# nucypher/SGFHE.jl

Hardware: AMD Instinct MI355X
Metric: bootstraps/sec (higher is better)
Workload: dtype i32

## Files before the change

sgfhe.jl_amd/csrc/engine.hip:

```cpp
#include "../../include/sgfhe_hip.h"

#include <math.h>
#include <stdio.h>
#include <stdlib.h>
#include <string.h>

#include <atomic>
#include <chrono>
#include <condition_variable>
#include <deque>
#include <memory>
#include <mutex>
#include <string>
#include <thread>
#include <type_traits>
#include <unordered_map>
#include <vector>

#include "kernels.h"
#include "host_plumbing.h"
#include "coalescer.h"
#include "circuit.h"

using namespace sgfhe;
// ... 74 lines not shown

struct SharedDev {
    int device = 0;
    std::mutex mu;
    std::vector<void *> mem;
    Coalescer co;
    std::atomic<unsigned> clones{0};
    void own(void *p) {
        std::lock_guard<std::mutex> g(mu);
        mem.push_back(p);
    }
    ~SharedDev() {
        (void)hipSetDevice(device);
        for (void *p : mem) (void)hipFree(p);
    }
};

struct sgfhe_ctx {
    sgfhe_params par;
    int device = 0;
    int logm = 0;
    uint32_t M = 0, n = 0;
    u128 Q = 0, B = 0;
    struct Basis {
        uint32_t npr = 0;
        uint32_t primes[NPR_MAX] = {};
        PrimeK *d_primes = nullptr;
        CrtConst *d_crt = nullptr;
        CrtConst h_crt;
        CrtLean *d_lean = nullptr;
        CrtLean h_lean;
        bool lean_rnd_ok = false;
        uint32_t pack_G = 1, pack_G_rnd = 0;
        int32_t *d_key = nullptr;
        size_t key_bytes = 0;
    } basis[2];
    int nb = 1, active = 0;
    uint32_t npr_max = 0;
    uint32_t tw_done = 0;
    std::string err;
    std::shared_ptr<SharedDev> shared;
    mutable std::recursive_mutex mu;
    hipStream_t stream = nullptr;
    hipStream_t stream2 = nullptr;
    hipEvent_t ev_fork = nullptr, ev_join = nullptr;
    hipEvent_t ev_done = nullptr;
    bool pending = false;
    hipStream_t stream_io = nullptr, stream_io2 = nullptr;
    std::vector<hipEvent_t> ev_pool;
    uint32_t *d_bad = nullptr;
    int32_t *d_tw = nullptr;
    int32_t *d_twq = nullptr;
    int32_t *d_pow = nullptr;
    int32_t tw_head[NPR_MAX][8] = {};
    uint32_t fused_min = 7;
    uint32_t split_max = 7;
    bool have_key = false;
    uint32_t chunk = 0, cap = 0, lanes = 2;
    bool rnd = false, rnd_ok = false;
    ChaChaKey rnd_key = {};
    uint32_t rnd_call = 0, last_call = 0;
    int64_t call_fixed = -1;
    const RndRow *gather_rows = nullptr;
    DevBuf<RndRow> d_rows;
    std::vector<RndRow> h_rows;
    uint32_t create_flags = 0;
    bool have_rns2 = false;
    Rns2Const rns2;
    struct Lane {
        uint64_t *dig = nullptr;
        uint32_t *yres = nullptr;
        uint32_t *ua = nullptr;
        int32_t *zpart = nullptr;
    } lane[2];
    bool small_padded = false;
    bool small_lanes = true;
    uint32_t small_lanes_max = 24;
    uint32_t crt1_max = 0;
    uint32_t small_max = 24;
    DevBuf<uint64_t> io_in, io_out;
    DevBuf<uint64_t, true> pin_in, pin_out;
    std::vector<uint64_t> co_buf;
    bool use_pin = true;
    DevBuf<uint64_t> circ_wires, circ_stage, circ_out;
    DevBuf<uint32_t> circ_tab;
    DevBuf<uint64_t> circ_ct;
    DevBuf<uint64_t> pack_lwe, pack_pdig, pack_wv;
    DevBuf<ulonglong2> pack_raw;
    DevBuf<uint32_t> pack_yg;
    DevBuf<ulonglong2> circ_raw;
    DevBuf<uint64_t> noise_tab, noise_lwe;
    bool timing = false;
    struct EvTriple { hipEvent_t e0, e1, e2; };
    std::vector<EvTriple> ev;
    double t_ext = 0, t_crt = 0;
    uint64_t n_ext = 0, n_crt = 0;
    uint32_t last_chunk = 0;
    struct EvPair { hipEvent_t e0, e1; uint64_t batch; };
    std::vector<EvPair> ev_call;
    double t_call = 0;
    uint64_t n_call = 0, boots_call = 0;
    uint32_t attr_done = 0;
};
enum : uint32_t { ATTR_EXTPROD = 1u, ATTR_SMALL = 2u, ATTR_SHORTPROD = 4u, ATTR_FUSED = 8u };
static constexpr size_t PIN_MAX_BYTES = (size_t)1 << 30;
static size_t pin_max_bytes() {
// ... 67 lines not shown
enum class ExtKind {
    Throughput,
    Small,
    Quarter,
    Fused
};
struct ExtForm {
    ExtKind kind;
    uint32_t cnt;
    bool quarter() const { return kind == ExtKind::Quarter || kind == ExtKind::Fused; }
};
ExtForm ext_form(const sgfhe_ctx *c, uint32_t mode, uint32_t cb, uint32_t cpad, bool has_zpart) {
    const bool small = cpad <= c->small_max && has_zpart;
    const uint32_t cnt = small && !c->small_padded ? cb : cpad;
    if (small && cnt >= c->fused_min && cnt <= fused_cap(c, mode)) return {ExtKind::Fused, cnt};
    if (small && quarter_ok(c, mode) && cnt <= c->split_max) return {ExtKind::Quarter, cnt};
    return {small ? ExtKind::Small : ExtKind::Throughput, cnt};
}

enum class CrtKind { Lean, LeanRnd, Acc2, Acc };
struct CrtForm {
    CrtKind kind;
    uint32_t np, nl;
    bool wide;
    bool rows;
    bool p87;
    bool one;
    bool quarter;
    uint32_t per_thread() const { return kind == CrtKind::Acc2 ? 2u : (kind == CrtKind::Acc || one) ? 1u : 4u; }
};
CrtForm crt_form(const sgfhe_ctx *c, uint32_t mode, uint32_t total, bool rows, bool quarter = false) {
    const sgfhe_ctx::Basis &S = cur(c);
    CrtForm f = {CrtKind::Acc, S.npr, S.h_lean.nl, false, false, false, false, quarter};
    if (quarter) {
        f.kind = (mode & MODE_RANDOM) ? CrtKind::LeanRnd : CrtKind::Lean;
        f.one = true;
    } else if (mode == 0u && S.h_lean.nl != 0) {
        f.kind = CrtKind::Lean;
        f.one = total <= c->crt1_max;
        f.p87 = !f.one && S.npr == 5 && S.h_lean.p87;
    } else if ((mode & ~MODE_WIDE) == MODE_RANDOM && S.lean_rnd_ok) {
        f.kind = CrtKind::LeanRnd;
        f.wide = (mode & MODE_WIDE) != 0;
        f.one = !f.wide && total <= c->crt1_max;
    } else if (mode == 0u) {
        f.kind = CrtKind::Acc2;
    }
    f.rows = rows && (f.kind == CrtKind::LeanRnd || f.kind == CrtKind::Acc);
    return f;
}

size_t lds_bytes(int logm, int npoly) { return (size_t)npoly * ((size_t)4 << logm); }
template <int LOGM> constexpr int ext_loge() { return LOGM <= EXT_LE3_MAX ? 3 : LOGE; }
template <int LOGM> constexpr int threads_of() { return NttGeom<LOGM, LOGE>::T; }


template <class F> int32_t with_logm(sgfhe_ctx *c, F &&f) {
    switch (c->logm) {
#define X(LM) case LM: return f(std::integral_constant<int, LM>{});
        X(6) X(7) X(8) X(9) X(10) X(11) X(12) X(13) X(14)
#undef X
    }
    return fail(c, SGFHE_ERR_UNSUPPORTED, "unsupported log2(m)");
}
template <class F> int32_t with_npr(sgfhe_ctx *c, uint32_t npr, F &&f) {
    switch (npr) {
#define X(NP) case NP: return f(std::integral_constant<int, NP>{});
        X(2) X(3) X(4) X(5) X(6) X(7)
#undef X
    }
    return fail(c, SGFHE_ERR_UNSUPPORTED, "unsupported number of RNS primes");
}
template <class F> void with_nl(uint32_t nl, F &&f) {
    switch (nl) {
    case 2: f(std::integral_constant<int, 2>{}); break;
    case 3: f(std::integral_constant<int, 3>{}); break;
    default: f(std::integral_constant<int, 4>{}); break;
    }
}
template <class F> void with_bool(bool b, F &&f) {
    if (b) f(std::true_type{});
    else f(std::false_type{});
}


int32_t launch_extprod(sgfhe_ctx *c, const sgfhe_ctx::Lane &L, const int32_t *keyk, uint32_t cpad,
                       uint32_t k, uint32_t mode, hipStream_t st) {
    return with_logm(c, [&](auto lm) -> int32_t {
        constexpr int LOGM = decltype(lm)::value, LE = ext_loge<LOGM>();
        const size_t lds = lds_bytes(LOGM, 2);
        if (!(c->attr_done & ATTR_EXTPROD)) {
            HIPCHK(c, hipFuncSetAttribute((const void *)k_extprod<LOGM, LE, false>,
                                          hipFuncAttributeMaxDynamicSharedMemorySize, (int)lds));
            HIPCHK(c, hipFuncSetAttribute((const void *)k_extprod<LOGM, LE, true>,
                                          hipFuncAttributeMaxDynamicSharedMemorySize, (int)lds));
            c->attr_done |= ATTR_EXTPROD;
        }
        with_bool(mode & MODE_WIDE, [&](auto wide) {
            hipLaunchKernelGGL((k_extprod<LOGM, LE, decltype(wide)::value>), dim3(cpad * cur(c).npr),
                               dim3(NttGeom<LOGM, LE>::T), lds, st, L.dig, keyk, L.yres, L.ua, cur(c).d_primes, k,
                               c->n, mode);
        });
        HIPCHK(c, hipGetLastError());
        return SGFHE_OK;
    });
}
// ... 683 lines not shown
    std::vector<int32_t> tw((size_t)NPR * 4 * M), twq, pwt;
    std::vector<PrimeK> pk(NPR);
    cc.npr = npr;
    for (int i = 0; i < NPR; i++) {
        const uint32_t p = S.primes[i];
        if ((uint32_t)i >= c->tw_done) {
        uint32_t psi = 0;
        for (uint32_t x = 2; x < 2000 && !psi; x++) {
            uint32_t g = powmod32(x, (p - 1) / (2 * M), p);
            if (powmod32(g, M, p) == p - 1) psi = g;
        }
        if (!psi) return fail(c, SGFHE_ERR_UNSUPPORTED, "no primitive 2m-th root of unity");
        const uint32_t ipsi = powmod32(psi, p - 2, p);
        int32_t *f = tw.data() + (size_t)(4 * i) * M, *v = f + M, *fp = f + 2 * M, *vp = f + 3 * M;
        const uint32_t R1m = (uint32_t)((1ull << 32) % p);
        std::vector<uint32_t> pf(M), pv(M);
        uint32_t pw = 1, ipw = 1;
        for (uint32_t t = 0; t < M; t++) {
            const uint32_t br = bitrev(t, logm);
            pf[br] = pw;
            pv[br] = ipw;
            f[br] = centre32(mulmod32(pw, R1m, p), p);
            v[br] = centre32(mulmod32(ipw, R1m, p), p);
            pw = mulmod32(pw, psi, p);
            ipw = mulmod32(ipw, ipsi, p);
        }
        fp[0] = fp[1] = vp[0] = vp[1] = 0;
        for (uint32_t j = 2; j < M; j++) {
            const uint32_t a = mulmod32(mulmod32(pf[j >> 1], pf[j], p), R1m, p);
            const uint32_t b = mulmod32(mulmod32(pv[j >> 1], pv[j], p), R1m, p);
            fp[j] = centre32((j & 1) ? (p - a) % p : a, p);
            vp[j] = centre32((j & 1) ? (p - b) % p : b, p);
        }
        if (M >= 16) {
            const uint32_t MS = M / 4;
            twq.assign((size_t)4 * M, 0);
            for (uint32_t q = 0; q < 4; q++)
                for (uint32_t jj = 1; jj < MS; jj++) {
                    const uint32_t mmq = 1u << (31 - __builtin_clz(jj)), J = 4 * mmq + q * mmq + (jj - mmq);
                    int32_t *blk = twq.data() + (size_t)q * M;
                    blk[jj] = f[J];
                    blk[MS + jj] = v[J];
                    blk[2 * MS + jj] = jj >= 2 ? fp[J] : 0;
                    blk[3 * MS + jj] = jj >= 2 ? vp[J] : 0;
                }
            HIPCHK(c, hipMemcpy(c->d_twq + (size_t)(4 * i) * M, twq.data(), (size_t)4 * M * sizeof(int32_t), hipMemcpyHostToDevice));
        }
        {
            pwt.resize((size_t)2 * M);
            uint32_t pe = 1;
            for (uint32_t e = 0; e < 2 * M; e++) { pwt[e] = centre32(mulmod32(pe, R1m, p), p); pe = mulmod32(pe, psi, p); }
            HIPCHK(c, hipMemcpy(c->d_pow + (size_t)(2 * i) * M, pwt.data(), (size_t)2 * M * sizeof(int32_t), hipMemcpyHostToDevice));
        }
        const int32_t head[8] = {f[1], M > 2 ? f[2] : 0, M > 2 ? f[3] : 0, M > 2 ? fp[2] : 0, M > 2 ? fp[3] : 0,
                                 v[1], M > 2 ? v[2] : 0, M > 2 ? v[3] : 0};
        memcpy(c->tw_head[i], head, sizeof head);
        }
        PrimeK &P = pk[i];
        memset(&P, 0, sizeof P);
        P.p = (int32_t)p;
        uint32_t inv = p;
        for (int it = 0; it < 5; it++) inv *= 2u - p * inv;
        P.pinv = inv;
        const uint32_t R1 = (uint32_t)((1ull << 32) % p);
        const uint32_t Rinv = powmod32(R1, p - 2, p);
        const uint32_t R2 = mulmod32(R1, R1, p);
        P.r1 = centre32(R1, p);
        P.r2 = centre32(R2, p);
        P.r3 = centre32(mulmod32(R2, R1, p), p);
        P.sR = centre32((p - mulmod32((uint32_t)(s % p), Rinv, p)) % p, p);
        {
            const u128 xmax = (B & 1) ? (B - 1) / 2 * 3 : B / 2 * 3;
            P.sRr = centre32((p - mulmod32((uint32_t)((s + xmax) % p), Rinv, p)) % p, p);
        }
        P.hoff = (i == NPR - 1) ? (p - 1) / 2 : 0;
        P.qmodp = centre32((uint32_t)(Q % p), p);
        uint32_t Mi = 1;
        for (int j = 0; j < NPR; j++)
            if (j != i) Mi = mulmod32(Mi, S.primes[j] % p, p);
        const uint32_t ei = powmod32(Mi, p - 2, p);
        const uint32_t minv = powmod32(M % p, p - 2, p);
        const uint32_t kappa = mulmod32(mulmod32(R2, minv, p), ei, p);
        P.kappaR = centre32(mulmod32(kappa, R1, p), p);
        P.minvR = centre32(mulmod32(minv, R1, p), p);
        P.invp = 1.0f / (float)p;
        P.twf = c->d_tw + (size_t)(4 * i) * M;
        P.twi = c->d_tw + (size_t)(4 * i + 1) * M;
        P.npr = npr;
        P.f1 = c->tw_head[i][0]; P.f2 = c->tw_head[i][1]; P.f3 = c->tw_head[i][2];
        P.fp2 = c->tw_head[i][3]; P.fp3 = c->tw_head[i][4];
        P.v1 = c->tw_head[i][5]; P.v2 = c->tw_head[i][6]; P.v3 = c->tw_head[i][7];
        P.twq = c->d_twq + (size_t)(4 * i) * M;
        P.pw = c->d_pow + (size_t)(2 * i) * M;
    }
    if (c->tw_done < npr) {
        const size_t off = (size_t)c->tw_done * 4 * M;
        HIPCHK(c, hipMemcpy(c->d_tw + off, tw.data() + off, ((size_t)npr * 4 * M - off) * sizeof(int32_t),
                            hipMemcpyHostToDevice));
        c->tw_done = npr;
    }
    HIPCHK(c, hipMalloc(&S.d_primes, NPR * sizeof(PrimeK)));
    c->shared->own(S.d_primes);
    HIPCHK(c, hipMemcpy(S.d_primes, pk.data(), NPR * sizeof(PrimeK), hipMemcpyHostToDevice));
    HIPCHK(c, hipMalloc(&S.d_crt, sizeof(CrtConst)));
    c->shared->own(S.d_crt);
    HIPCHK(c, hipMemcpy(S.d_crt, &cc, sizeof(CrtConst), hipMemcpyHostToDevice));
    HIPCHK(c, hipMalloc(&S.d_lean, sizeof(CrtLean)));
    c->shared->own(S.d_lean);
    HIPCHK(c, hipMemcpy(S.d_lean, &S.h_lean, sizeof(CrtLean), hipMemcpyHostToDevice));
    return SGFHE_OK;
}

int32_t build_constants(sgfhe_ctx *c) {
    const int logm = c->logm;
    const u128 Q = c->Q, B = c->B;

    uint32_t cand_primes[NPR_MAX];
    {
        int found = 0;
        for (uint64_t kk = ((1ull << 29) - 1) >> 15; kk > 0 && found < NPR_MAX; kk--) {
            uint32_t cand = (uint32_t)((kk << 15) + 1);
            if (cand < (1u << 29) && is_prime32(cand)) cand_primes[found++] = cand;
        }
        if (found < NPR_MAX) return fail(c, SGFHE_ERR_UNSUPPORTED, "could not find RNS primes");
    }
    const double log_mbq = logm + u128_log2(B) + u128_log2(Q);
    const double log_need = log2(5.0) + log_mbq + 0.001;
    auto fewest = [&](double target, double *have) {
        uint32_t npr = 0;
        double lh = 0;
        while (npr < NPR_MAX && (npr < 2 || lh < target)) lh += log2((double)cand_primes[npr++]);
        *have = lh;
        return lh >= target ? npr : 0u;
    };
    double have_det = 0, have_rnd = 0;
    const uint32_t npr_det = fewest(log_need, &have_det);
    if (!npr_det)
        return fail(c, SGFHE_ERR_UNSUPPORTED, "5 m B Q exceeds the product of the RNS primes");
    const bool rnd_width_ok = 2.0 * u128_log2(B) + 2.0 - u128_log2(Q) < 50.0;
    const uint32_t npr_rnd = fewest(log_need + 2.0, &have_rnd);
    const bool det_only = (c->create_flags & SGFHE_CTX_DETERMINISTIC_ONLY) != 0;
    c->nb = (!det_only && rnd_width_ok && npr_rnd > npr_det) ? 2 : 1;
    c->rnd_ok = rnd_width_ok && npr_rnd != 0 && (c->nb == 2 || npr_rnd == npr_det);
    c->npr_max = c->nb == 2 ? npr_rnd : npr_det;
    {
        const char *env = getenv("SGFHE_HOST_PIN");
        c->use_pin = !(env && env[0] == '0');
        env = getenv("SGFHE_SMALL_PADDED");
        c->small_padded = env && env[0] == '1';
        env = getenv("SGFHE_SMALL_LANES");
        if (env) { c->small_lanes = atoi(env) != 0; if (atoi(env) > 1) c->small_lanes_max = (uint32_t)atoi(env); }
        env = getenv("SGFHE_CRT1_GATES");
        c->crt1_max = (uint32_t)(env ? atoi(env) : 8) * 2u * c->M;
        if (c->logm >= 14) { c->small_max = 16; if (c->small_lanes_max > 16) c->small_lanes_max = 16; }
    }
    HIPCHK(c, hipMalloc(&c->d_tw, (size_t)c->npr_max * 4 * c->M * sizeof(int32_t)));
    c->shared->own(c->d_tw);
    HIPCHK(c, hipMalloc(&c->d_twq, (size_t)c->npr_max * 4 * c->M * sizeof(int32_t)));
    c->shared->own(c->d_twq);
    HIPCHK(c, hipMalloc(&c->d_pow, (size_t)c->npr_max * 2 * c->M * sizeof(int32_t)));
    c->shared->own(c->d_pow);
    {
        const char *env = getenv("SGFHE_SMALL_SPLIT");
        if (env) c->split_max = (uint32_t)atoi(env);
        env = getenv("SGFHE_SMALL_FUSED");
        if (env) c->fused_min = (uint32_t)atoi(env);
    }
    HIPCHK(c, hipMalloc(&c->d_bad, sizeof(uint32_t)));
    HIPCHK(c, hipMemset(c->d_bad, 0, sizeof(uint32_t)));
    for (int b = c->nb - 1; b >= 0; b--) {
        const bool big = b == c->nb - 1 && c->nb == 2;
        int32_t rc = build_basis(c, c->basis[b], big ? npr_rnd : npr_det, cand_primes, big ? have_rnd : have_det, log_mbq);
        if (rc) return rc;
    }
    c->active = 0;
    return SGFHE_OK;
}

int32_t key_begin(sgfhe_ctx *c) {
    if (c->shared.use_count() > 1)
        return fail(c, SGFHE_ERR_INVALID_ARG,
                    "the bootstrap key of this ctx is shared with clones (sgfhe_ctx_clone): destroy them before replacing it");
    c->active = c->nb - 1;
    return SGFHE_OK;
}
sgfhe_ctx::Basis &key_basis(sgfhe_ctx *c) { return c->basis[c->nb - 1]; }
void key_dirty(sgfhe_ctx *c) { c->have_key = false; }
int32_t key_finish(sgfhe_ctx *c, int32_t rc) {
    if (rc == SGFHE_OK && c->nb == 2) {
        const sgfhe_ctx::Basis &Bg = c->basis[1];
        sgfhe_ctx::Basis &Sm = c->basis[0];
        hipError_t e = hipSuccess;
        if (!Sm.d_key) {
            Sm.key_bytes = (size_t)c->n * Sm.npr * 8 * c->M * 4;
            e = hipMalloc(&Sm.d_key, Sm.key_bytes);
            if (e == hipSuccess) c->shared->own(Sm.d_key);
        }
        if (e == hipSuccess) {
            KeyFactors fac = {};
            for (uint32_t i = 0; i < Sm.npr; i++) {
                const uint32_t p = Sm.primes[i];
                uint32_t f = (uint32_t)((1ull << 32) % p);
                for (uint32_t j = Sm.npr; j < Bg.npr; j++) f = mulmod32(f, Bg.primes[j] % p, p);
                fac.f[i] = centre32(f, p);
            }
            const size_t total = Sm.key_bytes / 4;
            hipLaunchKernelGGL(k_key_derive, dim3((unsigned)((total + 255) / 256)), dim3(256), 0, c->stream,
                               Bg.d_key, Sm.d_key, Sm.d_primes, fac, Bg.npr, Sm.npr, (uint32_t)c->logm, total);
            e = hipGetLastError();
            if (e == hipSuccess) e = hipStreamSynchronize(c->stream);
        }
        if (e != hipSuccess) { rc = fail(c, SGFHE_ERR_HIP, hipGetErrorString(e)); c->have_key = false; }
    }
    c->active = mode_basis(c);
// ... 132 lines not shown
    {
        const char *env = getenv("SGFHE_COALESCE");
        if (env && env[0] == '0') c->shared->co.enabled = false;
    }
    const uint64_t m = p->m;
    if (p->ell != 2) return fail(c, SGFHE_ERR_UNSUPPORTED, "ell must be 2 (fhe.jl:576)");
    if (m < 64 || m > 16384 || (m & (m - 1)))
        return fail(c, SGFHE_ERR_UNSUPPORTED, "m must be a power of two in [2^6, 2^14]");
    if (p->r != 2 * m) return fail(c, SGFHE_ERR_INVALID_ARG, "r must equal 2 m (fhe.jl:62)");
    if (p->n == 0 || p->n > m / 4 || (p->n & (p->n - 1)))
        return fail(c, SGFHE_ERR_INVALID_ARG,
                    "n must be a power of two in [1, m / 4] (fhe.jl:45-46; extract, fhe.jl:585-590)");
    c->M = (uint32_t)m;
    c->n = (uint32_t)p->n;
    while ((1u << c->logm) < c->M) c->logm++;
    c->Q = ld128(p->Q);
    c->B = ld128(p->B);
    if (c->Q < 3 || (c->Q >> 94)) return fail(c, SGFHE_ERR_UNSUPPORTED, "Q must be in [3, 2^94)");
    if (c->B < 2 || (c->B >> 47)) return fail(c, SGFHE_ERR_UNSUPPORTED, "B must be in [2, 2^47)");
    {
        if (c->B * c->B < c->Q) return fail(c, SGFHE_ERR_INVALID_ARG, "B^2 must be >= Q");
    }
    if (ld128(p->DQ_tilde) >= c->Q) return fail(c, SGFHE_ERR_INVALID_ARG, "DQ_tilde must be < Q");
    int32_t rc = create_streams(c);
    if (rc) return rc;
    return build_constants(c);
}

int32_t sgfhe_ctx_clone(sgfhe_ctx *src, sgfhe_ctx **out) {
    if (!src || !out) return SGFHE_ERR_INVALID_ARG;
    *out = nullptr;
    SGFHE_LOCK(src);
    if (!src->have_key) return fail(src, SGFHE_ERR_NO_KEY, "ctx_clone: the ctx has no bootstrap key to share");
    if (hipSetDevice(src->device) != hipSuccess) return fail(src, SGFHE_ERR_NO_DEVICE, "ctx_clone: hipSetDevice failed");
    sgfhe_ctx *c = new (std::nothrow) sgfhe_ctx();
    if (!c) return fail(src, SGFHE_ERR_OOM, "out of host memory");
    *out = c;
    c->par = src->par;
    c->device = src->device;
    c->logm = src->logm;
    c->M = src->M;
    c->n = src->n;
    c->Q = src->Q;
    c->B = src->B;
    c->create_flags = src->create_flags;
    c->shared = src->shared;
    for (int b = 0; b < 2; b++) c->basis[b] = src->basis[b];
    c->nb = src->nb;
    c->npr_max = src->npr_max;
    c->tw_done = src->tw_done;
    c->d_tw = src->d_tw;
    c->d_twq = src->d_twq;
    c->d_pow = src->d_pow;
    memcpy(c->tw_head, src->tw_head, sizeof c->tw_head);
    c->rnd_ok = src->rnd_ok;
    c->have_rns2 = src->have_rns2;
    c->rns2 = src->rns2;
    c->have_key = true;
    c->chunk = src->chunk;
    c->lanes = src->lanes;
    c->small_max = src->small_max;
    c->small_lanes = src->small_lanes;
    c->small_lanes_max = src->small_lanes_max;
    c->small_padded = src->small_padded;
    c->crt1_max = src->crt1_max;
    c->split_max = src->split_max;
    c->fused_min = src->fused_min;
    c->use_pin = src->use_pin;
    hipStream_t skip[3] = {nullptr, nullptr, nullptr};
    const unsigned shift = c->shared->clones.fetch_add(1) % 4u + 1u;
    for (unsigned i = 0; i < shift % 4u; i++) (void)hipStreamCreateWithFlags(&skip[i], hipStreamNonBlocking);
    int32_t rc = create_streams(c);
    for (hipStream_t x : skip)
        if (x) (void)hipStreamDestroy(x);
    if (rc) return rc;
    HIPCHK(c, hipMalloc(&c->d_bad, sizeof(uint32_t)));
    HIPCHK(c, hipMemset(c->d_bad, 0, sizeof(uint32_t)));
    return SGFHE_OK;
}

static void free_circuit_buffers(sgfhe_ctx *c) {
    c->circ_wires.release();
    c->circ_stage.release();
    c->circ_out.release();
    c->circ_tab.release();
    c->circ_ct.release();
    c->circ_raw.release();
    c->noise_tab.release();
    c->noise_lwe.release();
    c->pack_lwe.release();
    c->pack_raw.release();
    c->pack_pdig.release();
    c->pack_yg.release();
    c->pack_wv.release();
}
static void free_io_buffers(sgfhe_ctx *c) {
    c->io_in.release();
    c->io_out.release();
    c->pin_in.release();
    c->pin_out.release();
}

extern "C++" template <typename T>
static int32_t circ_grow(sgfhe_ctx *c, DevBuf<T> &buf, size_t words) {
    if (buf.grow(words) == hipSuccess) return SGFHE_OK;
    return fail(c, SGFHE_ERR_OOM, "sgfhe_circuit_run: hipMalloc of " + std::to_string(words * sizeof(T)) +
// ... 1602 lines not shown
```

sgfhe.jl_amd/csrc/kernels.h:

```cpp
#pragma once

#include "ntt.h"

namespace sgfhe {

typedef unsigned __int128 u128;

constexpr int NPR_MAX = 7;
constexpr int LOGE = 4;

struct PrimeK {
    int32_t p;
    uint32_t pinv;
    int32_t sR;
    int32_t sRr;
    uint32_t hoff;
    int32_t r1, r2, r3;
    int32_t qmodp;
    int32_t kappaR;
    int32_t minvR;
    float invp;
    const int32_t *twf;
    const int32_t *twi;
    uint32_t npr;
    int32_t f1, f2, f3, fp2, fp3;
    int32_t v1, v2, v3;
    const int32_t *twq;
    const int32_t *pw;
};
__device__ __forceinline__ Mod mod_of(const PrimeK &P) { return Mod{P.p, -P.p, P.pinv}; }

typedef const PrimeK *__restrict__ PrimeSet;

constexpr int CRT_ALPHA_MAX = 6 * NPR_MAX + 2;

struct CrtConst {
    u128 Q, B;
    u128 c[NPR_MAX];
    u128 T[CRT_ALPHA_MAX];
    u128 offneg;
    u128 offneg_rnd;
    uint64_t xmax;
    u128 DQ;
    u128 halfQ;
    u128 roundthr;
    double invQ, invB;
    uint32_t c32[NPR_MAX][3];
    uint32_t Q32[3];
    alignas(16) uint32_t T32[CRT_ALPHA_MAX][4];
    double cd[NPR_MAX], Td[CRT_ALPHA_MAX], Bd;
    float invp[NPR_MAX];
    uint32_t npr;
    uint32_t logr;
    ulonglong2 dig0, digP, digN;
};

enum : uint32_t {
    MODE_PLAIN = 1u,
    MODE_NOACC = 2u,
    MODE_CANON = 4u,
    MODE_RANDOM = 16u,
    MODE_WIDE = 32u
};


__device__ __forceinline__ double u128_to_double(u128 x) {
    return (double)(uint64_t)(x >> 64) * 18446744073709551616.0 + (double)(uint64_t)x;
}
__device__ __forceinline__ u128 mul_u64_u128(uint64_t a, u128 b) {
    return (u128)a * (uint64_t)b + (((u128)(a * (uint64_t)(b >> 64))) << 64);
}
__device__ __forceinline__ u128 mod_wide(u128 x, u128 d, double inv, uint64_t *quot) {
    uint64_t q = (uint64_t)(u128_to_double(x) * inv);
    u128 r = x - mul_u64_u128(q, d);
#pragma unroll 1
    while ((__int128)r < 0) { r += d; q--; }
#pragma unroll 1
    while (r >= d) { r -= d; q++; }
    if (quot) *quot = q;
    return r;
}
// ... 173 lines not shown
    uint32_t q;
    int32_t wB, wP;
    __device__ __forceinline__ QuarterHead(uint32_t q_, const PrimeK &P)
        : q(q_), wB((q_ & 2) ? P.f3 : P.f2), wP((q_ & 2) ? P.fp3 : P.fp2) {}
    template <int MS>
    __device__ __forceinline__ int32_t point(const uint32_t *dl, const uint16_t *dh, uint32_t i, const PrimeK &P,
                                             const Mod &md, int32_t sRd) const {
        int32_t X[4];
#pragma unroll
        for (int t = 0; t < 4; t++)
            X[t] = digit_reduce(dl[i + t * MS] | ((uint64_t)dh[i + t * MS] << 32), md, sRd);
        const int32_t u = smont(X[2], P.f1, md);
        const int32_t a = (q & 2) ? X[0] - u : X[0] + u;
        const int32_t w = sredc((int64_t)X[1] * wB + (int64_t)X[3] * wP, md);
        return sred_floor((q & 1) ? a - w : a + w, md);
    }
};

template <int LOGM, int E>
__device__ __forceinline__ void rot_factors(int32_t (&dfac)[E], const PrimeK &P, uint32_t j, uint32_t q, int t) {
    constexpr uint32_t M = 1u << LOGM;
#pragma unroll
    for (int e = 0; e < E; e++) {
        const uint32_t sl = q * (M / 4) + (uint32_t)(E * t + e);
        const uint32_t br = __brev(sl) >> (32 - LOGM);
        dfac[e] = P.pw[(j * (2u * br + 1u)) & (2u * M - 1u)];
    }
}
__device__ __forceinline__ int32_t rot_centre(int32_t dfac, const PrimeK &P, const Mod &md) {
    return scentre(dfac - P.r1, md);
}

template <int NP>
__device__ __forceinline__ void quarter_residues(const int32_t *__restrict__ ypart, PrimeSet PS, uint32_t bc,
                                                 uint32_t i, uint32_t logm, uint32_t (&y)[NP]) {
    const uint32_t MS = (1u << logm) >> 2, jq = i & (MS - 1), qq = i >> (logm - 2);
#pragma unroll
    for (int q = 0; q < NP; q++) {
        const PrimeK P = PS[q];
        const Mod md = mod_of(P);
        const int32_t *yp = ypart + (((size_t)bc * NP + q) * 4) * MS + jq;
        int32_t r;
        if (qq & 1u) {
            const int32_t c1 = smont(yp[0] - yp[MS], P.v2, md), c3 = smont(yp[2 * MS] - yp[3 * MS], P.v3, md);
            r = (qq & 2u) ? smont(c1 - c3, P.v1, md) : c1 + c3;
        } else {
            const int32_t c0 = sred(yp[0] + yp[MS], md), c2 = sred(yp[2 * MS] + yp[3 * MS], md);
            r = (qq & 2u) ? smont(c0 - c2, P.v1, md) : c0 + c2;
        }
        y[q] = (uint32_t)r + handover_offset(P);
    }
}

constexpr int EXT_WAVES = 4;
constexpr int wide_split(int logm) { return logm >= 13 ? 2 : 4; }
constexpr int DET_SPLIT = 0;
constexpr int EXT_LE3_MAX = 9;
template <int LOGM, int LE, bool WIDE = false>
__global__ void __launch_bounds__((NttGeom<LOGM, LE>::T), (NttGeom<LOGM, LE>::T >= 256 ? EXT_WAVES : 1))
k_extprod(const uint64_t *__restrict__ dig, const int32_t *__restrict__ keyk,
          uint32_t *__restrict__ yres, const uint32_t *__restrict__ ua, PrimeSet PS, uint32_t k,
          uint32_t n, uint32_t mode) {
    using G = NttGeom<LOGM, LE>;
    constexpr int M = G::M, T = G::T, E = G::E;
    extern __shared__ __attribute__((aligned(16))) uint32_t lds[];
    int32_t *const z1 = reinterpret_cast<int32_t *>(lds) + M + threadIdx.x;

    const int tid = threadIdx.x;
    const uint32_t g = blockIdx.x;
    const uint32_t slot = g >> 3;
    const uint32_t npr = PS[0].npr;
    const uint32_t b = (slot / npr) * 8 + (g & 7);
    const uint32_t pi = slot % npr;
    const PrimeK P = PS[pi];
    const Mod md = mod_of(P);
    const uint32_t cpad = gridDim.x / npr;
    const BufRsrc rdig = make_rsrc(dig, cpad * 32u * (uint32_t)M);
    const BufRsrc rkey = make_rsrc(keyk, npr * 32u * (uint32_t)M);
#ifdef SGFHE_ABL_NO_YRES
    const BufRsrc ryres = make_rsrc(yres, 0u);
#else
    const BufRsrc ryres = make_rsrc(yres, cpad * npr * 8u * (uint32_t)M);
#endif

    const int32_t sRd = (mode & MODE_RANDOM) ? P.sRr : P.sR;
    constexpr int SPLIT = E == 16 ? (WIDE ? wide_split(LOGM) : DET_SPLIT) : 0;
    int64_t acc0[E];
#pragma unroll
    for (int e = 0; e < E; e++) { acc0[e] = 0; z1[e * T] = 0; }
#pragma unroll 1
    for (int ph = 0; ph < 4; ph++) {
        const int tid = (int)threadIdx.x + (int)opaque_zero();
        int32_t x[1][E];
        const uint32_t srec = (b * 2u + (uint32_t)(ph >> 1)) * 16u * (uint32_t)M;
        const uint32_t slo = srec + (uint32_t)(ph & 1) * 4u * (uint32_t)M;
        const uint32_t shi = srec + 8u * (uint32_t)M + (uint32_t)(ph & 1) * 2u * (uint32_t)M;
        const uint32_t vlo = 4u * (uint32_t)tid, vhi = 2u * (uint32_t)tid;
#pragma unroll
        for (int e = 0; e < E; e++) {
#ifdef SGFHE_ABL_NO_DIG
            x[0][e] = digit_reduce((uint64_t)(tid + e) * 0x9E3779B97F4Aull, md, sRd);
#else
            const uint32_t OL = (uint32_t)(4 * T * e), OH = (uint32_t)(2 * T * e);
            const uint32_t lo = buf_ld_u32(rdig, vlo + (OL & 4095u), slo + (OL & ~4095u));
            uint32_t hi = buf_ld_u16(rdig, vhi + (OH & 4095u), shi + (OH & ~4095u));
            if constexpr (WIDE)
                hi |= buf_ld_u8(rdig, (uint32_t)tid + ((uint32_t)(T * e) & 4095u),
                                srec + 12u * (uint32_t)M + (uint32_t)(ph & 1) * (uint32_t)M + ((uint32_t)(T * e) & ~4095u)) << 16;
            x[0][e] = digit_reduce(lo | ((uint64_t)hi << 32), md, sRd);
#endif
            if constexpr (SPLIT > 1)
                if ((e + 1) % (E / SPLIT) == 0 && e + 1 < E) __builtin_amdgcn_sched_barrier(0);
        }
        SGFHE_SYNC();

        const uint32_t skey = (pi * 8u + (uint32_t)ph * 2u) * 4u * (uint32_t)M;
        const uint32_t vkey = 4u * (uint32_t)E * (uint32_t)tid;
        int4 ka4[E / 4], kb4[E / 4];
        ntt_forward<LOGM, 1, LE>(x, lds, P.twf, tid, md);
#pragma unroll
        for (int h = 0; h < E / 4; h++) {
#ifdef SGFHE_ABL_NO_KEY
            ka4[h] = make_int4(tid, h, ph, 7), kb4[h] = make_int4(h, tid, 5, ph);
#else
            ka4[h] = buf_ld_i4(rkey, vkey + 16u * (uint32_t)h, skey);
            kb4[h] = buf_ld_i4(rkey, vkey + 16u * (uint32_t)h, skey + 4u * (uint32_t)M);
#endif
        }

        const Mod &mdp = md;
#pragma unroll
        for (int h = 0; h < E / 4; h++) {
            const int4 a = ka4[h], bq = kb4[h];
            const int32_t ka[4] = {a.x, a.y, a.z, a.w};
            const int32_t kb[4] = {bq.x, bq.y, bq.z, bq.w};
#pragma unroll
            for (int t = 0; t < 4; t++) {
                const int e = 4 * h + t;
                const int32_t u = x[0][e];
                acc0[e] += (int64_t)u * ka[t];
                int32_t *zp = reinterpret_cast<int32_t *>(lds) + M + e * T + tid;
                *zp += smont(u, kb[t], mdp);
            }
        }
    }
    int32_t z[2][E];
    constexpr bool WIDE0 = !inv_r4(LOGM) && LE == 4 && NttGeom<LOGM, LE>::SLAST_INV >= 0 &&
                           !(NttGeom<LOGM, LE>::RHO == 0 && NttGeom<LOGM, LE>::STOP == 0);
#pragma unroll
    for (int e = 0; e < E; e++) {
        const int32_t r0 = sredc(acc0[e], md);
        z[0][e] = WIDE0 ? r0 : sred(r0, md);
        z[1][e] = sred(z1[e * T], md);
    }
    SGFHE_SYNC();
    ntt_inverse<LOGM, 2, LE, WIDE0>(z, lds, P.twi, tid, md);

    const uint32_t sy0 = (b * 2u * npr + pi) * 4u * (uint32_t)M;
    const uint32_t sy1 = sy0 + npr * 4u * (uint32_t)M;
    const uint32_t vout = 4u * (uint32_t)tid;
    if (mode & MODE_PLAIN) {
#pragma unroll
        for (int c = 0; c < 2; c++)
#pragma unroll
            for (int e = 0; e < E; e++)
                buf_st_u32(ryres, vout + ((uint32_t)(4 * T * e) & 4095u),
                              (c ? sy1 : sy0) + ((uint32_t)(4 * T * e) & ~4095u),
                              condsub(sfull(z[c][e], md) + P.hoff, (uint32_t)P.p));
        return;
    }
    const uint32_t j = ua[(size_t)b * n + k];
    const uint32_t yoff = handover_offset(P);
    lds_store<LOGM, 2, LE, G::STOP>(z, lds, tid);
    SGFHE_SYNC();
    {
        constexpr uint32_t LOWMASK = (1u << G::STOP) - 1u;
        const uint32_t s0 = ((uint32_t)tid - j) & (2 * M - 1);
        const uint32_t lowswz = swz<LE>(s0 & LOWMASK);
        const uint32_t h0 = s0 >> G::STOP;
#pragma unroll
        for (int e = 0; e < E; e++) {
            const uint32_t he = h0 + e;
            const uint32_t hipart = (he & (E - 1)) << G::STOP;
            const uint32_t addr = hipart ^ lowswz ^ (G::STOP >= 9 ? 0u : swz_bits<LE>(hipart));
            const uint32_t smask = 0u - ((he >> LE) & 1u);
            const uint32_t yoe = yoff - smask;
#pragma unroll
            for (int c = 0; c < 2; c++) {
                const uint32_t v = lds[c * M + addr];
                const uint32_t y = (v ^ smask) + (yoe - (uint32_t)z[c][e]);
                buf_st_u32(ryres, vout + ((uint32_t)(4 * T * e) & 4095u),
                              (c ? sy1 : sy0) + ((uint32_t)(4 * T * e) & ~4095u), y);
            }
        }
    }
}

struct U96 {
    uint32_t w0, w1, w2;
};
__device__ __forceinline__ void mad96(U96 &a, uint32_t y, const uint32_t (&c)[3]) {
    const uint64_t p0 = (uint64_t)y * c[0] + a.w0;
    const uint64_t p1 = (uint64_t)y * c[1] + a.w1 + (p0 >> 32);
    a.w0 = (uint32_t)p0;
    a.w1 = (uint32_t)p1;
    a.w2 = y * c[2] + a.w2 + (uint32_t)(p1 >> 32);
}
template <int NP>
__device__ __forceinline__ U96 crt_reduce(const uint32_t (&y)[NP], const CrtConst *__restrict__ CC,
                                          bool have_old, ulonglong2 d) {
    float f = 0.f;
    double Sd = 0.0;
#pragma unroll
    for (int q = 0; q < NP; q++) {
        f += (float)y[q] * CC->invp[q];
#ifndef SGFHE_ABL_CRT_NOSD
        Sd += (double)y[q] * CC->cd[q];
#endif
    }
    const int alpha = (int)f;
    const uint4 tv = *reinterpret_cast<const uint4 *>(CC->T32[alpha]);
    U96 a = {tv.x, tv.y, tv.z};
    Sd += CC->Td[alpha];
#pragma unroll
    for (int q = 0; q < NP; q++) mad96(a, y[q], CC->c32[q]);
    if (have_old) {
        const uint64_t B = (uint64_t)CC->B;
        const uint32_t h0 = (uint32_t)d.y, h1 = (uint32_t)(d.y >> 32);
        const uint32_t b0 = (uint32_t)B, b1 = (uint32_t)(B >> 32);
        const uint64_t p0 = (uint64_t)h0 * b0 + a.w0 + (uint32_t)d.x;
        const uint64_t p1 = (uint64_t)h0 * b1 + (uint64_t)h1 * b0 + a.w1 + (uint32_t)(d.x >> 32) + (p0 >> 32);
        a.w0 = (uint32_t)p0;
        a.w1 = (uint32_t)p1;
        a.w2 += h1 * b1 + (uint32_t)(p1 >> 32);
#ifndef SGFHE_ABL_CRT_NOSD
        Sd += (double)d.y * CC->Bd + (double)d.x;
#endif
    }
    {
        const uint64_t q1 = (uint64_t)(Sd * CC->invQ);
        const uint32_t qa = (uint32_t)q1, qb = (uint32_t)(q1 >> 32);
        const uint64_t m0 = (uint64_t)qa * CC->Q32[0];
        const uint64_t m1 = (uint64_t)qa * CC->Q32[1] + (uint64_t)qb * CC->Q32[0] + (m0 >> 32);
        const uint32_t m2 = qa * CC->Q32[2] + qb * CC->Q32[1] + (uint32_t)(m1 >> 32);
        const uint64_t r0 = (uint64_t)a.w0 - (uint32_t)m0;
        const uint64_t r1 = (uint64_t)a.w1 - (uint32_t)m1 - ((r0 >> 32) & 1u);
        a.w2 = a.w2 - m2 - (uint32_t)((r1 >> 32) & 1u);
        a.w0 = (uint32_t)r0;
// ... 1544 lines not shown
```

Baseline: 2177.

## Fold negacyclic rotation into NTT domain via precomputed (X^j-1) twiddle table

The external-product kernel used to finish with an LDS store, a barrier, and a rotated re-read that formed X^j*z - z in the coefficient domain. Now each NTT-domain value is multiplied pointwise by a precomputed (psi^e - 1) factor before the inverse NTT, so the output can be stored directly. The factors are loaded from a new per-prime table laid out in rows. This removes an LDS round trip and a sync at the cost of extra global table reads and Montgomery multiplies, and it drops the WIDE0 lazy-reduction path.

```diff
diff --git a/sgfhe.jl_amd/csrc/engine.hip b/sgfhe.jl_amd/csrc/engine.hip
--- a/sgfhe.jl_amd/csrc/engine.hip
+++ b/sgfhe.jl_amd/csrc/engine.hip
@@ -150,6 +150,7 @@
     int32_t *d_tw = nullptr;
     int32_t *d_twq = nullptr;
     int32_t *d_pow = nullptr;
+    int32_t *d_rot = nullptr;
     int32_t tw_head[NPR_MAX][8] = {};
     uint32_t fused_min = 7;
     uint32_t split_max = 7;
@@ -323,6 +324,7 @@
 
 size_t lds_bytes(int logm, int npoly) { return (size_t)npoly * ((size_t)4 << logm); }
 template <int LOGM> constexpr int ext_loge() { return LOGM <= EXT_LE3_MAX ? 3 : LOGE; }
+uint32_t rot_row_words(int logm) { return 1u << (logm <= EXT_LE3_MAX ? 3 : LOGE); }
 template <int LOGM> constexpr int threads_of() { return NttGeom<LOGM, LOGE>::T; }
 
 
@@ -1112,6 +1114,16 @@
             for (uint32_t e = 0; e < 2 * M; e++) { pwt[e] = centre32(mulmod32(pe, R1m, p), p); pe = mulmod32(pe, psi, p); }
             HIPCHK(c, hipMemcpy(c->d_pow + (size_t)(2 * i) * M, pwt.data(), (size_t)2 * M * sizeof(int32_t), hipMemcpyHostToDevice));
         }
+        {
+            const uint32_t E = rot_row_words(logm), rows = 2 * M / E;
+            pwt.assign((size_t)2 * M + E, centre32(R1m, p));
+            uint32_t pe = 1;
+            for (uint32_t e = 0; e < 2 * M; e++) {
+                pwt[(size_t)(e % rows) * E + e / rows] = centre32(mulmod32((pe + p - 1) % p, R1m, p), p);
+                pe = mulmod32(pe, psi, p);
+            }
+            HIPCHK(c, hipMemcpy(c->d_rot + (size_t)i * (2 * M + E), pwt.data(), pwt.size() * sizeof(int32_t), hipMemcpyHostToDevice));
+        }
         const int32_t head[8] = {f[1], M > 2 ? f[2] : 0, M > 2 ? f[3] : 0, M > 2 ? fp[2] : 0, M > 2 ? fp[3] : 0,
                                  v[1], M > 2 ? v[2] : 0, M > 2 ? v[3] : 0};
         memcpy(c->tw_head[i], head, sizeof head);
@@ -1152,6 +1164,7 @@
         P.v1 = c->tw_head[i][5]; P.v2 = c->tw_head[i][6]; P.v3 = c->tw_head[i][7];
         P.twq = c->d_twq + (size_t)(4 * i) * M;
         P.pw = c->d_pow + (size_t)(2 * i) * M;
+        P.rot = c->d_rot + (size_t)i * (2 * M + rot_row_words(logm));
     }
     if (c->tw_done < npr) {
         const size_t off = (size_t)c->tw_done * 4 * M;
@@ -1220,6 +1233,8 @@
     c->shared->own(c->d_twq);
     HIPCHK(c, hipMalloc(&c->d_pow, (size_t)c->npr_max * 2 * c->M * sizeof(int32_t)));
     c->shared->own(c->d_pow);
+    HIPCHK(c, hipMalloc(&c->d_rot, (size_t)c->npr_max * (2 * c->M + rot_row_words(c->logm)) * sizeof(int32_t)));
+    c->shared->own(c->d_rot);
     {
         const char *env = getenv("SGFHE_SMALL_SPLIT");
         if (env) c->split_max = (uint32_t)atoi(env);
@@ -1458,6 +1473,7 @@
     c->d_tw = src->d_tw;
     c->d_twq = src->d_twq;
     c->d_pow = src->d_pow;
+    c->d_rot = src->d_rot;
     memcpy(c->tw_head, src->tw_head, sizeof c->tw_head);
     c->rnd_ok = src->rnd_ok;
     c->have_rns2 = src->have_rns2;
diff --git a/sgfhe.jl_amd/csrc/kernels.h b/sgfhe.jl_amd/csrc/kernels.h
--- a/sgfhe.jl_amd/csrc/kernels.h
+++ b/sgfhe.jl_amd/csrc/kernels.h
@@ -27,6 +27,7 @@
     int32_t v1, v2, v3;
     const int32_t *twq;
     const int32_t *pw;
+    const int32_t *rot;
 };
 __device__ __forceinline__ Mod mod_of(const PrimeK &P) { return Mod{P.p, -P.p, P.pinv}; }
 
@@ -306,6 +307,23 @@
     }
 }
 
+template <int LOGM, int LE>
+struct RotRow {
+    static constexpr int E = 1 << LE, LOGROWS = LOGM + 1 - LE;
+    BufRsrc rrot;
+    uint32_t j, row, h4;
+    __device__ __forceinline__ RotRow(const PrimeK &P, uint32_t j_, int tid, bool plain)
+        : rrot(make_rsrc(P.rot, (8u << LOGM) + 4u * E)), j(j_) {
+        const uint32_t jd = j * (2u * (__brev((uint32_t)tid) >> (32 - (LOGM - LE))) + 1u);
+        row = plain ? (8u << LOGM) : (jd & ((1u << LOGROWS) - 1u)) * (4u * E);
+        h4 = (jd >> LOGROWS) << 2;
+    }
+    __device__ __forceinline__ int32_t load(int e) const {
+        const uint32_t se4 = (j * (__brev((uint32_t)e) >> (32 - LE))) << 2;
+        return (int32_t)buf_ld_u32(rrot, row | ((h4 + se4) & (4u * E - 4u)), 0u);
+    }
+};
+
 constexpr int EXT_WAVES = 4;
 constexpr int wide_split(int logm) { return logm >= 13 ? 2 : 4; }
 constexpr int DET_SPLIT = 0;
@@ -338,6 +356,7 @@
 #endif
 
     const int32_t sRd = (mode & MODE_RANDOM) ? P.sRr : P.sR;
+    const uint32_t j = ua[(size_t)b * n + k];
     constexpr int SPLIT = E == 16 ? (WIDE ? wide_split(LOGM) : DET_SPLIT) : 0;
     int64_t acc0[E];
 #pragma unroll
@@ -398,17 +417,16 @@
             }
         }
     }
+    const RotRow<LOGM, LE> rot(P, j, tid + (int)opaque_zero(), (mode & MODE_PLAIN) != 0);
     int32_t z[2][E];
-    constexpr bool WIDE0 = !inv_r4(LOGM) && LE == 4 && NttGeom<LOGM, LE>::SLAST_INV >= 0 &&
-                           !(NttGeom<LOGM, LE>::RHO == 0 && NttGeom<LOGM, LE>::STOP == 0);
 #pragma unroll
     for (int e = 0; e < E; e++) {
-        const int32_t r0 = sredc(acc0[e], md);
-        z[0][e] = WIDE0 ? r0 : sred(r0, md);
-        z[1][e] = sred(z1[e * T], md);
+        const int32_t f = rot.load(e);
+        z[0][e] = smont(sredc(acc0[e], md), f, md);
+        z[1][e] = smont(z1[e * T], f, md);
     }
     SGFHE_SYNC();
-    ntt_inverse<LOGM, 2, LE, WIDE0>(z, lds, P.twi, tid, md);
+    ntt_inverse<LOGM, 2, LE>(z, lds, P.twi, tid, md);
 
     const uint32_t sy0 = (b * 2u * npr + pi) * 4u * (uint32_t)M;
     const uint32_t sy1 = sy0 + npr * 4u * (uint32_t)M;
@@ -423,31 +441,13 @@
                               condsub(sfull(z[c][e], md) + P.hoff, (uint32_t)P.p));
         return;
     }
-    const uint32_t j = ua[(size_t)b * n + k];
     const uint32_t yoff = handover_offset(P);
-    lds_store<LOGM, 2, LE, G::STOP>(z, lds, tid);
-    SGFHE_SYNC();
-    {
-        constexpr uint32_t LOWMASK = (1u << G::STOP) - 1u;
-        const uint32_t s0 = ((uint32_t)tid - j) & (2 * M - 1);
-        const uint32_t lowswz = swz<LE>(s0 & LOWMASK);
-        const uint32_t h0 = s0 >> G::STOP;
-#pragma unroll
-        for (int e = 0; e < E; e++) {
-            const uint32_t he = h0 + e;
-            const uint32_t hipart = (he & (E - 1)) << G::STOP;
-            const uint32_t addr = hipart ^ lowswz ^ (G::STOP >= 9 ? 0u : swz_bits<LE>(hipart));
-            const uint32_t smask = 0u - ((he >> LE) & 1u);
-            const uint32_t yoe = yoff - smask;
-#pragma unroll
-            for (int c = 0; c < 2; c++) {
-                const uint32_t v = lds[c * M + addr];
-                const uint32_t y = (v ^ smask) + (yoe - (uint32_t)z[c][e]);
-                buf_st_u32(ryres, vout + ((uint32_t)(4 * T * e) & 4095u),
-                              (c ? sy1 : sy0) + ((uint32_t)(4 * T * e) & ~4095u), y);
-            }
-        }
-    }
+#pragma unroll
+    for (int c = 0; c < 2; c++)
+#pragma unroll
+        for (int e = 0; e < E; e++)
+            buf_st_u32(ryres, vout + ((uint32_t)(4 * T * e) & 4095u),
+                          (c ? sy1 : sy0) + ((uint32_t)(4 * T * e) & ~4095u), (uint32_t)z[c][e] + yoff);
 }
 
 struct U96 {
```

After: 2105. -3.3%, worse.

## Pair digit phases in external product with parked NTT and joint reduction

Applied to the files above, without the earlier changes.

Restructures the external-product accumulation loop so two digit phases are processed per pass. The first phase's forward-NTT output is parked in LDS and combined with the second's in a single 64-bit multiply-add pair, followed by one Montgomery reduction per output per pair. This replaces the 64-bit accumulator plus a per-element LDS read-modify-write with smont for the second component. The goal is to cut reductions and LDS traffic. In exchange the kernel drops the WIDE0 inverse-NTT path, adds an LDS park store and reload, and puts an extra sred between reductions that may change numeric bounds.

```diff
diff --git a/sgfhe.jl_amd/csrc/kernels.h b/sgfhe.jl_amd/csrc/kernels.h
--- a/sgfhe.jl_amd/csrc/kernels.h
+++ b/sgfhe.jl_amd/csrc/kernels.h
@@ -318,7 +318,7 @@
     using G = NttGeom<LOGM, LE>;
     constexpr int M = G::M, T = G::T, E = G::E;
     extern __shared__ __attribute__((aligned(16))) uint32_t lds[];
-    int32_t *const z1 = reinterpret_cast<int32_t *>(lds) + M + threadIdx.x;
+    int32_t *const park = reinterpret_cast<int32_t *>(lds) + M + threadIdx.x;
 
     const int tid = threadIdx.x;
     const uint32_t g = blockIdx.x;
@@ -339,76 +339,76 @@
 
     const int32_t sRd = (mode & MODE_RANDOM) ? P.sRr : P.sR;
     constexpr int SPLIT = E == 16 ? (WIDE ? wide_split(LOGM) : DET_SPLIT) : 0;
-    int64_t acc0[E];
-#pragma unroll
-    for (int e = 0; e < E; e++) { acc0[e] = 0; z1[e * T] = 0; }
+    int32_t s0[E], s1[E];
+#pragma unroll
+    for (int e = 0; e < E; e++) s0[e] = s1[e] = 0;
 #pragma unroll 1
-    for (int ph = 0; ph < 4; ph++) {
-        const int tid = (int)threadIdx.x + (int)opaque_zero();
+    for (int pr = 0; pr < 2; pr++) {
         int32_t x[1][E];
-        const uint32_t srec = (b * 2u + (uint32_t)(ph >> 1)) * 16u * (uint32_t)M;
-        const uint32_t slo = srec + (uint32_t)(ph & 1) * 4u * (uint32_t)M;
-        const uint32_t shi = srec + 8u * (uint32_t)M + (uint32_t)(ph & 1) * 2u * (uint32_t)M;
-        const uint32_t vlo = 4u * (uint32_t)tid, vhi = 2u * (uint32_t)tid;
-#pragma unroll
-        for (int e = 0; e < E; e++) {
+        int tid = 0;
+#pragma unroll 1
+        for (int hb = 0; hb < 2; hb++) {
+            const int ph = 2 * pr + hb;
+            tid = (int)threadIdx.x + (int)opaque_zero();
+            const uint32_t srec = (b * 2u + (uint32_t)(ph >> 1)) * 16u * (uint32_t)M;
+            const uint32_t slo = srec + (uint32_t)(ph & 1) * 4u * (uint32_t)M;
+            const uint32_t shi = srec + 8u * (uint32_t)M + (uint32_t)(ph & 1) * 2u * (uint32_t)M;
+            const uint32_t vlo = 4u * (uint32_t)tid, vhi = 2u * (uint32_t)tid;
+#pragma unroll
+            for (int e = 0; e < E; e++) {
 #ifdef SGFHE_ABL_NO_DIG
-            x[0][e] = digit_reduce((uint64_t)(tid + e) * 0x9E3779B97F4Aull, md, sRd);
+                x[0][e] = digit_reduce((uint64_t)(tid + e) * 0x9E3779B97F4Aull, md, sRd);
 #else
-            const uint32_t OL = (uint32_t)(4 * T * e), OH = (uint32_t)(2 * T * e);
-            const uint32_t lo = buf_ld_u32(rdig, vlo + (OL & 4095u), slo + (OL & ~4095u));
-            uint32_t hi = buf_ld_u16(rdig, vhi + (OH & 4095u), shi + (OH & ~4095u));
-            if constexpr (WIDE)
-                hi |= buf_ld_u8(rdig, (uint32_t)tid + ((uint32_t)(T * e) & 4095u),
-                                srec + 12u * (uint32_t)M + (uint32_t)(ph & 1) * (uint32_t)M + ((uint32_t)(T * e) & ~4095u)) << 16;
-            x[0][e] = digit_reduce(lo | ((uint64_t)hi << 32), md, sRd);
+                const uint32_t OL = (uint32_t)(4 * T * e), OH = (uint32_t)(2 * T * e);
+                const uint32_t lo = buf_ld_u32(rdig, vlo + (OL & 4095u), slo + (OL & ~4095u));
+                uint32_t hi = buf_ld_u16(rdig, vhi + (OH & 4095u), shi + (OH & ~4095u));
+                if constexpr (WIDE)
+                    hi |= buf_ld_u8(rdig, (uint32_t)tid + ((uint32_t)(T * e) & 4095u),
+                                    srec + 12u * (uint32_t)M + (uint32_t)(ph & 1) * (uint32_t)M + ((uint32_t)(T * e) & ~4095u)) << 16;
+                x[0][e] = digit_reduce(lo | ((uint64_t)hi << 32), md, sRd);
 #endif
-            if constexpr (SPLIT > 1)
-                if ((e + 1) % (E / SPLIT) == 0 && e + 1 < E) __builtin_amdgcn_sched_barrier(0);
+                if constexpr (SPLIT > 1)
+                    if ((e + 1) % (E / SPLIT) == 0 && e + 1 < E) __builtin_amdgcn_sched_barrier(0);
+            }
+            SGFHE_SYNC();
+
+            ntt_forward<LOGM, 1, LE>(x, lds, P.twf, tid, md);
+            if (hb == 0) {
+#pragma unroll
+                for (int e = 0; e < E; e++) park[e * T] = x[0][e];
+            }
         }
-        SGFHE_SYNC();
-
-        const uint32_t skey = (pi * 8u + (uint32_t)ph * 2u) * 4u * (uint32_t)M;
+        const uint32_t skey = (pi * 8u + (uint32_t)pr * 4u) * 4u * (uint32_t)M;
         const uint32_t vkey = 4u * (uint32_t)E * (uint32_t)tid;
-        int4 ka4[E / 4], kb4[E / 4];
-        ntt_forward<LOGM, 1, LE>(x, lds, P.twf, tid, md);
 #pragma unroll
         for (int h = 0; h < E / 4; h++) {
+            int32_t kk[4][4];
+#pragma unroll
+            for (int r = 0; r < 4; r++) {
 #ifdef SGFHE_ABL_NO_KEY
-            ka4[h] = make_int4(tid, h, ph, 7), kb4[h] = make_int4(h, tid, 5, ph);
+                const int4 v = make_int4(tid, h, pr, 7 + r);
 #else
-            ka4[h] = buf_ld_i4(rkey, vkey + 16u * (uint32_t)h, skey);
-            kb4[h] = buf_ld_i4(rkey, vkey + 16u * (uint32_t)h, skey + 4u * (uint32_t)M);
+                const int4 v = buf_ld_i4(rkey, vkey + 16u * (uint32_t)h, skey + (uint32_t)r * 4u * (uint32_t)M);
 #endif
-        }
-
-        const Mod &mdp = md;
-#pragma unroll
-        for (int h = 0; h < E / 4; h++) {
-            const int4 a = ka4[h], bq = kb4[h];
-            const int32_t ka[4] = {a.x, a.y, a.z, a.w};
-            const int32_t kb[4] = {bq.x, bq.y, bq.z, bq.w};
+                kk[r][0] = v.x; kk[r][1] = v.y; kk[r][2] = v.z; kk[r][3] = v.w;
+            }
 #pragma unroll
             for (int t = 0; t < 4; t++) {
                 const int e = 4 * h + t;
-                const int32_t u = x[0][e];
-                acc0[e] += (int64_t)u * ka[t];
-                int32_t *zp = reinterpret_cast<int32_t *>(lds) + M + e * T + tid;
-                *zp += smont(u, kb[t], mdp);
+                const int32_t ua = park[e * T], ub = x[0][e];
+                s0[e] += sredc((int64_t)ua * kk[0][t] + (int64_t)ub * kk[2][t], md);
+                s1[e] += sredc((int64_t)ua * kk[1][t] + (int64_t)ub * kk[3][t], md);
             }
         }
     }
     int32_t z[2][E];
-    constexpr bool WIDE0 = !inv_r4(LOGM) && LE == 4 && NttGeom<LOGM, LE>::SLAST_INV >= 0 &&
-                           !(NttGeom<LOGM, LE>::RHO == 0 && NttGeom<LOGM, LE>::STOP == 0);
 #pragma unroll
     for (int e = 0; e < E; e++) {
-        const int32_t r0 = sredc(acc0[e], md);
-        z[0][e] = WIDE0 ? r0 : sred(r0, md);
-        z[1][e] = sred(z1[e * T], md);
+        z[0][e] = sred(s0[e], md);
+        z[1][e] = sred(s1[e], md);
     }
     SGFHE_SYNC();
-    ntt_inverse<LOGM, 2, LE, WIDE0>(z, lds, P.twi, tid, md);
+    ntt_inverse<LOGM, 2, LE>(z, lds, P.twi, tid, md);
 
     const uint32_t sy0 = (b * 2u * npr + pi) * 4u * (uint32_t)M;
     const uint32_t sy1 = sy0 + npr * 4u * (uint32_t)M;
```

After: 2152 before, 2069 after. 3.8% lower.
